# noorgme/Decentralised-Verification-and-Distributed-Execution-of-Large-Scale-Video-Diffusion-Models

Measured on AMD Instinct MI355X. Metric: denoising steps/sec, Zeroscope-XL 24f@1024x576 (CFG UNet3D forward + guidance + DDIM), higher is better.
Workload: dtype f16

## Files before the change

### decentralised-verification-and-distributed-execution-of-large-scale-video-diffusion-models_amd/_lib.py

```python
from __future__ import annotations

import ctypes as C
import os

_HERE = os.path.dirname(os.path.abspath(__file__))
LIB_PATH = os.environ.get("VDX_LIB_PATH") or os.path.join(_HERE, "libvdx_hip.so")


class GemmArgs(C.Structure):
    _fields_ = [
        ("a", C.c_void_p), ("a2", C.c_void_p), ("w", C.c_void_p), ("bias", C.c_void_p),
        ("bias2", C.c_void_p), ("residual", C.c_void_p), ("out", C.c_void_p),
        ("M", C.c_int32), ("N", C.c_int32), ("K", C.c_int32), ("mode", C.c_int32),
        ("c1", C.c_int32), ("c2", C.c_int32),
        ("lda", C.c_int32), ("lda2", C.c_int32), ("ldo", C.c_int32), ("ldr", C.c_int32),
        ("h_in", C.c_int32), ("w_in", C.c_int32), ("h_out", C.c_int32), ("w_out", C.c_int32),
        ("stride", C.c_int32), ("upsample", C.c_int32), ("frames", C.c_int32), ("hw", C.c_int32),
        ("rows_per_bias2", C.c_int32), ("ldb2", C.c_int32), ("epilogue", C.c_int32),
        ("row_begin", C.c_int32), ("row_end", C.c_int32),
        ("ksplit", C.c_int32), ("wset_rows", C.c_int32), ("workspace", C.c_void_p), ("wset_bias", C.c_void_p),
        ("workspace_bytes", C.c_size_t), ("pad_mode", C.c_int32),
    ]


class ClipPreprocessArgs(C.Structure):
    _fields_ = [
        ("frames", C.c_void_p), ("x_bounds", C.c_void_p), ("x_coeffs", C.c_void_p), ("y_bounds", C.c_void_p),
        ("y_coeffs", C.c_void_p), ("out", C.c_void_p), ("out_u8", C.c_void_p),
        ("frame_pitch", C.c_size_t), ("row_pitch", C.c_int32), ("F", C.c_int32), ("H", C.c_int32), ("W", C.c_int32),
        ("kx", C.c_int32), ("ky", C.c_int32), ("band", C.c_int32), ("span", C.c_int32), ("ldo", C.c_int32),
    ]


class TomeArgs(C.Structure):
    _fields_ = [
        ("src_idx", C.c_void_p), ("dst_idx", C.c_void_p), ("inv", C.c_void_p), ("node_max", C.c_void_p),
        ("node_idx", C.c_void_p), ("slot", C.c_void_p), ("off", C.c_void_p), ("items", C.c_void_p),
        ("n_img", C.c_int32), ("S", C.c_int32), ("n_src", C.c_int32), ("n_dst", C.c_int32), ("r", C.c_int32), ("C", C.c_int32),
    ]


_vp, _i, _f, _sz = C.c_void_p, C.c_int, C.c_float, C.c_size_t

SIGNATURES = {
    "vdx_last_error": (C.c_char_p, []),
    "vdx_version": (_i, []),
    "vdx_build_flags": (_i, []),
    "vdx_gemm_f16": (_i, [C.POINTER(GemmArgs), _vp]),
    "vdx_gemm_plan": (_i, [C.POINTER(GemmArgs), C.POINTER(C.c_int32), C.POINTER(C.c_int32)]),
    "vdx_gemm_kernel_name": (_i, [C.POINTER(GemmArgs), C.c_char_p, _sz]),
    "vdx_gemm_plan_ksplit": (_i, [C.POINTER(GemmArgs), C.POINTER(C.c_int32), C.POINTER(C.c_int32), C.POINTER(C.c_size_t)]),
    "vdx_softmax_rows_f16": (_i, [_vp, _i, _i, _i, _f, _vp]),
    "vdx_rows_to_u8_frames": (_i, [_vp, _i, _sz, _vp, _vp]),
    "vdx_im2col_in_f16": (_i, [_vp, _vp, _i, _i, _i, _i, _i, _i, _vp]),
    "vdx_rows_to_ncfhw_f16": (_i, [_vp, _i, _vp, _i, _i, _i, _i, _i, _vp]),
    "vdx_silu_f16": (_i, [_vp, _vp, _sz, _vp]),
    "vdx_groupnorm_workspace": (_sz, [_i, _i, _i, _i]),
    "vdx_groupnorm_f16": (_i, [_vp, _i, _i, _vp, _i, _i, _vp, _vp, _f, _i, _i, _i, _i, _vp, _i, _vp, _vp]),
    "vdx_groupnorm_workspace_part": (_sz, [_i, _i, _i, _i, _i]),
    "vdx_groupnorm_part_f16": (_i, [_vp, _i, _i, _vp, _i, _i, _vp, _vp, _f, _i, _i, _i, _i, _vp, _i, _vp, _i, _vp]),
    "vdx_groupnorm_fold_linear_f16": (_i, [_vp, _i, _i, _vp, _vp, _f, _i, _i, _i, _vp, _i, _vp, _vp, _i, _vp, _vp, _vp]),
    "vdx_groupnorm_stats_f16": (_i, [_vp, _i, _i, _vp, _i, _i, _vp, _vp, _f, _i, _i, _i, _vp, _i, C.POINTER(_sz), _vp]),
    "vdx_conv3x3_gn_supported": (_i, [_i, _i, _i]),
    "vdx_conv3x3_gn_preferred": (_i, [_i, _i, _i, _i, _i, _i]),
    "vdx_conv3x3_gn_f16": (_i, [_vp, _i, _vp, _i, _i, _i, _vp, _vp, _vp, _vp, _i, _i, _vp, _i, _vp, _i, _i, _i, _i, _i, _vp]),
    "vdx_tconv_gn_supported": (_i, [_i, _i, _i]),
    "vdx_tconv_gn_preferred": (_i, [_i, _i, _i, _i, _i]),
    "vdx_tconv_gn_f16": (_i, [_vp, _i, _vp, _vp, _vp, _vp, _i, _vp, _i, _i, _i, _i, _i, _i, _vp]),
    "vdx_layernorm_f16": (_i, [_vp, _i, _vp, _vp, _f, _i, _i, _vp, _i, _vp]),
    "vdx_flash_attn_f16": (_i, [_vp, _i, _vp, _i, _vp, _i, _vp, _i, _i, _i, _i, _i, _i, _i, _f, _i, _vp]),
    "vdx_flash_attn_rows_f16": (_i, [_vp, _i, _vp, _i, _vp, _i, _vp, _i, _i, _i, _i, _i, _i, _i, _f, _i, _vp]),
    "vdx_timestep_embedding_f16": (_i, [_vp, _vp, _i, _i, _vp]),
    "vdx_gelu_f16": (_i, [_vp, _vp, _sz, _vp]),
    "vdx_temporal_attn_f16": (_i, [_vp, _i, _vp, _i, _i, _i, _i, _i, _f, _vp]),
    "vdx_ff_block_supported": (_i, [_i]),
    "vdx_ff_block_pack_bytes": (_sz, [_i]),
    "vdx_ff_block_f16": (_i, [_vp, _i, _vp, _f, _vp, _i, _i, _i, _vp]),
    "vdx_ff_block_proj_pack_bytes": (_sz, [_i]),
    "vdx_ff_block_proj_f16": (_i, [_vp, _i, _vp, _f, _vp, _i, _i, _vp, _vp, _i, _i, _i, _vp]),
    "vdx_cross_attn_block_supported": (_i, [_i, _i]),
    "vdx_cross_attn_block_pack_bytes": (_sz, [_i]),
    "vdx_cross_attn_block_kv_bytes": (_sz, [_i]),
    "vdx_cross_attn_block_f16": (_i, [_vp, _i, _vp, _vp, _i, _f, _vp, _i, _i, _i, _i, _vp]),
    "vdx_temporal_attn_block_supported": (_i, [_i, _i]),
    "vdx_temporal_attn_block_wqkv_bytes": (_sz, [_i]),
    "vdx_temporal_attn_block_wo_bytes": (_sz, [_i]),
    "vdx_temporal_attn_block_f16": (_i, [_vp, _i, _vp, _vp, _f, _vp, _vp, _vp, _vp, _i, _i, _i, _i, _i, _f, _vp]),
    "vdx_temporal_attn_block2_supported": (_i, [_i, _i]),
    "vdx_temporal_attn_block2_pack_bytes": (_sz, [_i]),
    "vdx_temporal_attn_block2_f16": (_i, [_vp, _i, _vp, _f, _vp, _i, _i, _i, _i, _i, _vp]),
    "vdx_comm_unique_id": (_i, [_vp]),
    "vdx_comm_init": (_i, [_vp, _i, _i, C.POINTER(_vp)]),
    "vdx_comm_destroy": (_i, [_vp]),
    "vdx_allgather_shard": (_i, [_vp, _vp, _vp, _sz, _vp]),
    "vdx_halo_exchange": (_i, [_vp, _vp, _sz, _i, _vp, _sz, _i, _vp]),
    "vdx_ipc_export": (_i, [_vp, _vp, C.POINTER(_sz)]),
    "vdx_ipc_open": (_i, [_vp, _sz, C.POINTER(_vp)]),
    "vdx_ipc_close": (_i, [_vp, _sz]),
    "vdx_peer_gather": (_i, [_vp, C.POINTER(_vp), _i, _sz, _vp]),
    "vdx_set_reserved_cus": (_i, [_i]),
    "vdx_reserved_cus": (_i, []),
    "vdx_persistent_grid_cus": (_i, []),
    "vdx_probe_mfma_f16": (_i, [_vp, _sz, _i, C.POINTER(C.c_double), _vp]),
    "vdx_probe_occupancy_hog": (_i, [_i, _i, _i, _vp]),
    "vdx_cfg_input_f16": (_i, [_vp, _vp, _f, _vp, _i, _i, _i, _vp]),
    "vdx_cfg_ddim_step_f16": (_i, [_vp, _vp, _vp, _f, _f, _f, _f, _f, _sz, _vp]),
    "vdx_ddim_step_f16": (_i, [_vp, _vp, _vp, _f, _f, _f, _f, _sz, _vp]),
    "vdx_cfg_dpm_step_f16": (_i, [_vp, _vp, _vp, _vp, _vp, _f, _f, _f, _f, _f, _f, _f, _sz, _vp]),
    "vdx_dpm_step_f16": (_i, [_vp, _vp, _vp, _vp, _vp, _f, _f, _f, _f, _f, _f, _sz, _vp]),
    "vdx_blend_accumulate_f16": (_i, [_vp, _vp, _vp, _vp, _i, _i, _i, _i, _i, _vp]),
    "vdx_blend_finalize_f32": (_i, [_vp, _vp, _vp, _i, _i, _i, _vp]),
    "vdx_clip_preprocess_u8": (_i, [C.POINTER(ClipPreprocessArgs), _vp]),
    "vdx_clip_vision_embed_f16": (_i, [_vp, _i, _vp, _vp, _vp, _vp, _f, _i, _i, _i, _i, _vp, _i, _vp]),
# ... 156 lines not shown
```

### decentralised-verification-and-distributed-execution-of-large-scale-video-diffusion-models_amd/csrc/norm.hip

```cpp
#include "vdx_common.h"

static int gn_rows_for(int n_samples, int rows_per_sample, int min_blocks) {
    int rows = 128;
    while (rows > 8 && (long long)n_samples * ((rows_per_sample + rows - 1) / rows) < min_blocks) rows >>= 1;
    return rows;
}
static int gn_stat_rows(int n_samples, int rows_per_sample) { return gn_rows_for(n_samples, rows_per_sample, 256); }

struct GnP {
    const f16 *x, *x2;
    int c1, c2, ldx, ldx2;
    int C, G, cpg, nvec, krows;
    int n_samples, rps, nslabs, slab_rows;
    int apply_rows;
    float* partial;
    float* ab;
};

__device__ __forceinline__ f16x8 gn_load(const GnP& p, size_t row, int cv) {
    const int c = cv * 8;
    const f16* src = c < p.c1 ? p.x + row * p.ldx + c : p.x2 + row * p.ldx2 + (c - p.c1);
    return *(const f16x8*)src;
}

struct Moments {
    float n, mean, m2;
};
__device__ __forceinline__ Moments merge(const Moments a, const Moments b) {
    if (b.n == 0.f) return a;
    if (a.n == 0.f) return b;
    const float n = a.n + b.n, d = b.mean - a.mean;
    return Moments{n, a.mean + d * (b.n / n), a.m2 + b.m2 + d * d * (a.n * b.n / n)};
}

__global__ void gn_partial_kernel(const GnP p) {
    extern __shared__ float lds[];
    const int tid = threadIdx.x;
    const int sample = blockIdx.y, slab = blockIdx.x;
    const int cv = tid % p.nvec, rsub = tid / p.nvec;
    float k[8], s[8], ss[8];
#pragma unroll
    for (int j = 0; j < 8; ++j) k[j] = s[j] = ss[j] = 0.f;
    const int r_end = min(p.rps, (slab + 1) * p.slab_rows);
    const size_t base = (size_t)sample * p.rps;
    int cnt = 0;
    int r = slab * p.slab_rows + rsub;
    auto acc = [&](const f16x8 v) {
#pragma unroll
        for (int j = 0; j < 8; ++j) {
            const float f = (float)v[j] - k[j];
            s[j] += f;
            ss[j] += f * f;
        }
// ... 108 lines not shown
__global__ void gn_apply_kernel(const GnP p, f16* y, int ldy) {
    const int tid = threadIdx.x;
    const int sample = blockIdx.y, slab = blockIdx.x;
    const int cv = tid % p.nvec, rsub = tid / p.nvec;
    float a[8], b[8];
    const float* ab = p.ab + ((size_t)sample * p.C + cv * 8) * 2;
#pragma unroll
    for (int j = 0; j < 8; ++j) {
        a[j] = ab[2 * j];
        b[j] = ab[2 * j + 1];
    }
    const int r_end = min(p.rps, (slab + 1) * p.apply_rows);
    const size_t base = (size_t)sample * p.rps;
    for (int r = slab * p.apply_rows + rsub; r < r_end; r += p.krows) {
        const size_t row = base + r;
        const f16x8 v = gn_load(p, row, cv);
        f16x8 o;
#pragma unroll
        for (int j = 0; j < 8; ++j) {
            float f = (float)v[j] * a[j] + b[j];
            if (SILU) f = silu_f(f);
            o[j] = (f16)f;
        }
        *(f16x8*)(y + row * ldy + cv * 8) = o;
    }
}

static int gn_threads(int nvec, int* krows) {
    int k = nvec >= 256 ? 1 : (256 + nvec - 1) / nvec;
    *krows = k;
    return k * nvec;
}

extern "C" size_t vdx_groupnorm_workspace_part(int n_samples, int rows_per_sample, int C, int G, int partition_samples) {
    const int rows = gn_stat_rows(partition_samples > 0 ? partition_samples : n_samples, rows_per_sample);
    const size_t nslabs = (rows_per_sample + rows - 1) / rows;
    return ((((size_t)n_samples * nslabs * G * 3 + 3) & ~(size_t)3) + (size_t)n_samples * C * 2) * sizeof(float);
}
extern "C" size_t vdx_groupnorm_workspace(int n_samples, int rows_per_sample, int C, int G) {
    return vdx_groupnorm_workspace_part(n_samples, rows_per_sample, C, G, 0);
}

extern "C" int vdx_groupnorm_part_f16(const void* x, int c1, int ldx, const void* x2, int c2, int ldx2,
                                      const void* gamma, const void* beta, float eps, int G,
                                      int n_samples, int rows_per_sample, int silu, void* y, int ldy,
                                      void* workspace, int partition_samples, vdx_stream_t stream);
extern "C" int vdx_groupnorm_f16(const void* x, int c1, int ldx, const void* x2, int c2, int ldx2,
                                 const void* gamma, const void* beta, float eps, int G,
                                 int n_samples, int rows_per_sample, int silu, void* y, int ldy,
                                 void* workspace, vdx_stream_t stream) {
    return vdx_groupnorm_part_f16(x, c1, ldx, x2, c2, ldx2, gamma, beta, eps, G, n_samples, rows_per_sample, silu, y, ldy,
                                  workspace, 0, stream);
}
static int gn_run(const void* x, int c1, int ldx, const void* x2, int c2, int ldx2,
                  const void* gamma, const void* beta, float eps, int G,
                  int n_samples, int rows_per_sample, int silu, void* y, int ldy,
                  void* workspace, int partition_samples, bool stats_only, GnP& p, vdx_stream_t stream) {
    VDX_CHECK(x && gamma && beta && (y || stats_only) && workspace, "groupnorm: null pointer");
    const int C = c1 + c2;
    VDX_CHECK(c1 > 0 && c1 % 8 == 0 && c2 % 8 == 0, "groupnorm: c1=%d c2=%d must be multiples of 8", c1, c2);
    VDX_CHECK((c2 == 0) == (x2 == nullptr), "groupnorm: x2/c2 mismatch");
    VDX_CHECK(G > 0 && C % G == 0, "groupnorm: C=%d not divisible by G=%d", C, G);
    VDX_CHECK(ldx % 8 == 0 && ldy % 8 == 0 && (c2 == 0 || ldx2 % 8 == 0), "groupnorm: leading dims must be multiples of 8");
    VDX_CHECK(n_samples > 0 && rows_per_sample > 0, "groupnorm: empty input");
    VDX_CHECK(C / 8 <= 1024, "groupnorm: C=%d too wide", C);
    p.x = (const f16*)x; p.x2 = (const f16*)x2; p.c1 = c1; p.c2 = c2; p.ldx = ldx; p.ldx2 = ldx2;
    p.C = C; p.G = G; p.cpg = C / G; p.nvec = C / 8;
    p.n_samples = n_samples; p.rps = rows_per_sample;
    p.slab_rows = gn_stat_rows(partition_samples > 0 ? partition_samples : n_samples, rows_per_sample);
    p.apply_rows = gn_rows_for(n_samples, rows_per_sample, 1024);
    p.nslabs = (rows_per_sample + p.slab_rows - 1) / p.slab_rows;
    p.partial = (float*)workspace;
    p.ab = p.partial + (((size_t)n_samples * p.nslabs * G * 3 + 3) & ~(size_t)3);
    const int nt = gn_threads(p.nvec, &p.krows);
    hipStream_t st = (hipStream_t)stream;
    dim3 grid(p.nslabs, n_samples);
    hipLaunchKernelGGL(gn_partial_kernel, grid, dim3(nt), (2 * (size_t)p.krows * C + p.krows + 2 * (size_t)G * p.krows) * sizeof(float), st, p);
    const int nsg = n_samples * G;
    hipLaunchKernelGGL(gn_finalize_kernel, dim3((nsg + 3) / 4), dim3(256), 0, st, p, (const f16*)gamma, (const f16*)beta, eps);
    if (stats_only) return vdx_launch_status("vdx_groupnorm_f16 (statistics)");
    dim3 agrid((rows_per_sample + p.apply_rows - 1) / p.apply_rows, n_samples);
    if (silu)
        hipLaunchKernelGGL(gn_apply_kernel<true>, agrid, dim3(nt), 0, st, p, (f16*)y, ldy);
    else
        hipLaunchKernelGGL(gn_apply_kernel<false>, agrid, dim3(nt), 0, st, p, (f16*)y, ldy);
    return vdx_launch_status("vdx_groupnorm_f16");
}
extern "C" int vdx_groupnorm_part_f16(const void* x, int c1, int ldx, const void* x2, int c2, int ldx2,
                                      const void* gamma, const void* beta, float eps, int G,
                                      int n_samples, int rows_per_sample, int silu, void* y, int ldy,
                                      void* workspace, int partition_samples, vdx_stream_t stream) {
    GnP p;
    return gn_run(x, c1, ldx, x2, c2, ldx2, gamma, beta, eps, G, n_samples, rows_per_sample, silu, y, ldy, workspace,
                  partition_samples, false, p, stream);
}

extern "C" int vdx_groupnorm_stats_f16(const void* x, int c1, int ldx, const void* x2, int c2, int ldx2, const void* gamma,
                                       const void* beta, float eps, int G, int n_samples, int rows_per_sample, void* workspace,
                                       int partition_samples, size_t* scale_shift_offset, vdx_stream_t stream) {
    VDX_CHECK(scale_shift_offset, "groupnorm_stats: null pointer");
    GnP p;
    if (const int rc = gn_run(x, c1, ldx, x2, c2, ldx2, gamma, beta, eps, G, n_samples, rows_per_sample, 0, nullptr, 0, workspace,
                              partition_samples, true, p, stream))
        return rc;
    *scale_shift_offset = (size_t)((const char*)p.ab - (const char*)workspace);
    return 0;
}

__global__ void gn_fold_kernel(const float* ab, const f16* beta, const f16* w, const f16* bias, int C, int N, int n_samples,
                               f16* w_out, float* bias_out) {
    const int lane = threadIdx.x & 63;
    const long long sn = (long long)blockIdx.x * (blockDim.x >> 6) + (threadIdx.x >> 6);
    if (sn >= (long long)n_samples * N) return;
    const int sample = (int)(sn / N), n = (int)(sn % N);
    const float* abs_ = ab + (size_t)sample * C * 2;
    const f16* wr = w + (size_t)n * C;
    f16* wo = w_out + ((size_t)sample * N + n) * C;
    float acc = 0.f;
    for (int c = lane; c < C; c += 64) {
        const float a = abs_[2 * c], b = abs_[2 * c + 1], wv = (float)wr[c], be = (float)beta[c];
        const f16 w16 = (f16)(wv * a);
        wo[c] = w16;
        const float mean = a != 0.f ? (be - b) / a : 0.f;
        acc += wv * be - (float)w16 * mean;
    }
    acc = wave_sum(acc);
    if (lane == 0) bias_out[(size_t)sample * N + n] = acc + (bias ? (float)bias[n] : 0.f);
}

extern "C" int vdx_groupnorm_fold_linear_f16(const void* x, int C, int ldx, const void* gamma, const void* beta, float eps, int G,
                                             int n_samples, int rows_per_sample, void* workspace, int partition_samples,
                                             const void* w, const void* bias, int N, void* w_out, void* bias_out,
                                             vdx_stream_t stream) {
    VDX_CHECK(w && w_out && bias_out, "groupnorm_fold_linear: null pointer");
    VDX_CHECK(N > 0 && (long long)n_samples * N < (1ll << 31), "groupnorm_fold_linear: bad N");
    GnP p;
    if (const int rc = gn_run(x, C, ldx, nullptr, 0, 0, gamma, beta, eps, G, n_samples, rows_per_sample, 0, nullptr, 0, workspace,
                              partition_samples, true, p, stream))
        return rc;
    const long long waves = (long long)n_samples * N;
    hipLaunchKernelGGL(gn_fold_kernel, dim3((unsigned)((waves + 3) / 4)), dim3(256), 0, (hipStream_t)stream, p.ab, (const f16*)beta,
                       (const f16*)w, (const f16*)bias, C, N, n_samples, (f16*)w_out, (float*)bias_out);
    return vdx_launch_status("vdx_groupnorm_fold_linear_f16");
}

template <int NV>
__global__ __launch_bounds__(256) void layernorm_kernel(const f16* x, int ldx, const f16* gamma, const f16* beta,
                                                         float eps, int M, int C, f16* y, int ldy) {
    const int lane = threadIdx.x & 63;
    const int row = blockIdx.x * 4 + (threadIdx.x >> 6);
    if (row >= M) return;
    const int nvec = C >> 3;
    const f16* xr = x + (size_t)row * ldx;
    f16x8 v[NV];
    float s = 0.f;
#pragma unroll
    for (int i = 0; i < NV; ++i) {
        const int cv = lane + 64 * i;
        if (cv < nvec) {
            v[i] = *(const f16x8*)(xr + cv * 8);
#pragma unroll
            for (int j = 0; j < 8; ++j) s += (float)v[i][j];
        }
    }
    const float mean = wave_sum(s) / (float)C;
    float q = 0.f;
#pragma unroll
    for (int i = 0; i < NV; ++i) {
        if (lane + 64 * i < nvec) {
#pragma unroll
            for (int j = 0; j < 8; ++j) {
                const float d = (float)v[i][j] - mean;
                q += d * d;
            }
        }
    }
    const float rstd = rsqrtf(wave_sum(q) / (float)C + eps);
    f16* yr = y + (size_t)row * ldy;
#pragma unroll
    for (int i = 0; i < NV; ++i) {
        const int cv = lane + 64 * i;
        if (cv < nvec) {
            const f16x8 g = *(const f16x8*)(gamma + cv * 8);
            const f16x8 b = *(const f16x8*)(beta + cv * 8);
            f16x8 o;
#pragma unroll
            for (int j = 0; j < 8; ++j) o[j] = (f16)(((float)v[i][j] - mean) * rstd * (float)g[j] + (float)b[j]);
            *(f16x8*)(yr + cv * 8) = o;
        }
    }
}

template <int CTRL>
__device__ __forceinline__ float dpp_add(float v) {
    return v + __builtin_bit_cast(float, __builtin_amdgcn_update_dpp(0, __builtin_bit_cast(int, v), CTRL, 0xF, 0xF, false));
}
// ... 191 lines not shown
```

### decentralised-verification-and-distributed-execution-of-large-scale-video-diffusion-models_amd/ops.py

```python
from __future__ import annotations

import contextlib
import ctypes as C
from typing import NamedTuple, Optional, Tuple

import torch

from . import _lib
from ._lib import GemmArgs, VdxError
from .frames import is_packed

PLAIN, CONV3X3, TCONV3 = 0, 1, 2
EPI_GEGLU = 1


def _stream() -> int:
    return torch.cuda.current_stream().cuda_stream


def _p(t: Optional[torch.Tensor], name: str, dtype=torch.float16) -> Optional[int]:
    if t is None:
        return None
    if not t.is_cuda:
        raise VdxError(f"{name}: expected a GPU tensor (the denoising path has no CPU fallback)")
# ... 372 lines not shown


def clip_preprocess(frames, out=None, return_u8=False):
    F, H, W = check_u8_frames(frames, "clip_preprocess")
    if pillow_resizes_vertically_first(H, W, CLIP_IMAGE):
        frames, H = resize_u8(frames, CLIP_IMAGE, W, "bilinear"), CLIP_IMAGE
    dev = frames.device
    xb, xk, _ = _clip_table(W, dev)
    yb, yk, yb_host = _clip_table(H, dev)
    band = CLIP_BAND
    while band > 1 and clip_band_span(yb_host, band) * CLIP_IMAGE * 3 > CLIP_LDS_MAX:
        band //= 2
    span = clip_band_span(yb_host, band)
    if span * CLIP_IMAGE * 3 > CLIP_LDS_MAX:
        raise VdxError(f"clip_preprocess: H={H} needs {span} input rows per output row (more than LDS holds)")
    out, ldo = _out(out, F * 49, 3072, frames, "clip_preprocess")
    u8 = torch.empty((F, CLIP_IMAGE, CLIP_IMAGE, 3), dtype=torch.uint8, device=dev) if return_u8 else None
    a = _lib.ClipPreprocessArgs()
    a.frames, a.frame_pitch, a.row_pitch = _u8_args(frames)
    a.out, a.out_u8 = _p(out, "out"), (u8.data_ptr() if u8 is not None else None)
    a.x_bounds, a.x_coeffs, a.y_bounds, a.y_coeffs = xb.data_ptr(), xk.data_ptr(), yb.data_ptr(), yk.data_ptr()
    a.F, a.H, a.W = F, H, W
    a.kx, a.ky, a.band, a.span, a.ldo = xk.shape[1], yk.shape[1], band, span, ldo
    _launch("vdx_clip_preprocess_u8", C.byref(a))
    return (out, u8) if return_u8 else out


def clip_vision_embed(patch, class_emb, pos_emb, gamma, beta, *, F, seq_pad, eps=1e-5, out=None):
    r, D, ldp = _rows(patch, "patch")
    P = pos_emb.shape[0] - 1
    if r < F * P or pos_emb.shape[1] != D or class_emb.numel() != D or gamma.numel() != D or beta.numel() != D:
        raise VdxError(f"clip_vision_embed: patch [{r}][{D}], pos {tuple(pos_emb.shape)}: shapes do not match F={F}")
    if seq_pad <= P or not pos_emb.is_contiguous():
        raise VdxError(f"clip_vision_embed: seq_pad={seq_pad} must exceed {P} patches; pos_emb contiguous")
    out, ldo = _out(out, F * seq_pad, D, patch, "clip_vision_embed")
    _launch("vdx_clip_vision_embed_f16", _p(patch, "patch"), ldp, _p(class_emb, "class_emb"), _p(pos_emb, "pos_emb"),
            _p(gamma, "gamma"), _p(beta, "beta"), float(eps), F, P, seq_pad, D, _p(out, "out"), ldo)
    return out


def clip_cosine_score(img, txt):
    F, D, ldi = _rows(img, "img")
    if txt.numel() != D or not txt.is_contiguous():
        raise VdxError(f"clip_cosine_score: text embedding has {txt.numel()} values, images {D}")
    if F == 0:
        raise VdxError("clip_cosine_score: no frames")
    per = torch.empty(F, dtype=torch.float32, device=img.device)
    mean = torch.empty(1, dtype=torch.float32, device=img.device)
    _launch("vdx_clip_cosine_score_f16", _p(img, "img"), ldi, _p(txt, "txt"), F, D, _p(per, "per_frame", torch.float32),
            _p(mean, "mean", torch.float32))
    return mean, per


def groupnorm(x, gamma, beta, *, groups, n_samples, rows_per_sample, eps, silu_act, x2=None, out=None, partition_samples=0):
    r, c1, ldx = _rows(x, "x")
    c2, ldx2 = 0, 0
    M = n_samples * rows_per_sample
    if r < M:
        raise VdxError(f"groupnorm: x has {r} rows, need {M}")
    if x2 is not None:
        r2, c2, ldx2 = _rows(x2, "x2")
        if r2 < M:
            raise VdxError(f"groupnorm: x2 has {r2} rows, need {M}")
    Cc = c1 + c2
    if gamma.numel() != Cc or beta.numel() != Cc:
        raise VdxError(f"groupnorm: gamma/beta size {gamma.numel()} != C={Cc}")
    out, ldy = _out(out, M, Cc, x, "groupnorm")
    need = _lib.load().vdx_groupnorm_workspace_part(n_samples, rows_per_sample, Cc, groups, partition_samples)
    ws = _scratch(_GN_WS, x.device, need, torch.uint8, 1 << 20)
    _launch("vdx_groupnorm_part_f16", _p(x, "x"), c1, ldx, _p(x2, "x2"), c2, ldx2, _p(gamma, "gamma"), _p(beta, "beta"),
            float(eps), groups, n_samples, rows_per_sample, int(bool(silu_act)), _p(out, "out"), ldy, ws.data_ptr(),
            partition_samples)
    return out


def conv3x3_gn_preferred(c1: int, c2: int, N: int, n_img: int, h: int, w: int) -> bool:
    return bool(_lib.load().vdx_conv3x3_gn_preferred(c1, c2, N, n_img, h, w))


def conv3x3_gn_supported(c1: int, c2: int, N: int) -> bool:
    return bool(_lib.load().vdx_conv3x3_gn_supported(c1, c2, N))


def conv3x3_gn(x, gamma, beta, w, *, x2=None, bias=None, bias2=None, rows_per_bias2=0, residual=None, groups, n_img, h, wd, eps,
               partition_samples=0, out=None):
    r, c1, ldx = _rows(x, "x")
    S = h * wd
    M = n_img * S
    c2 = ldx2 = 0
    if x2 is not None:
        r2, c2, ldx2 = _rows(x2, "x2")
        if r2 < M:
            raise VdxError(f"conv3x3_gn: x2 has {r2} rows, need {M}")
    Cc = c1 + c2
    N, K = w.shape
    if r < M or K != 9 * Cc or gamma.numel() != Cc or beta.numel() != Cc or not w.is_contiguous():
        raise VdxError(f"conv3x3_gn: x [{r}][{c1}] (+{c2}), w [{N}][{K}], gamma {gamma.numel()}, M = {M}: shapes do not match")
    if not conv3x3_gn_supported(c1, c2, N):
        raise VdxError(f"conv3x3_gn: c1={c1}, c2={c2}, N={N} not supported")
    if bias is not None and bias.numel() != N:
        raise VdxError(f"conv3x3_gn: bias has {bias.numel()} elements, N={N}")
    ldb2 = _covers(bias2, M, N, "conv3x3_gn", "bias2", rows_per_bias2)
    ldr = _covers(residual, M, N, "conv3x3_gn", "residual")
    out, ldo = _out(out, M, N, x, "conv3x3_gn")
    need = _lib.load().vdx_groupnorm_workspace_part(n_img, S, Cc, groups, partition_samples)
    ws = _scratch(_GN_WS, x.device, need, torch.uint8, 1 << 20)
# ... 1722 lines not shown
```

### include/vdx.h

```cpp
#ifndef VDX_H
#define VDX_H
#include <stddef.h>
#include <stdint.h>

#ifdef __cplusplus
extern "C" {
#endif

typedef void* vdx_stream_t;

const char* vdx_last_error(void);
int vdx_version(void);
int vdx_build_flags(void);

enum { VDX_GEMM_PLAIN = 0, VDX_GEMM_CONV3X3 = 1, VDX_GEMM_TCONV3 = 2 };
enum { VDX_EPI_GEGLU = 1 };

typedef struct vdx_gemm_args {
    const void* a;
    const void* a2;
    const void* w;
    const void* bias;
    const void* bias2;
    const void* residual;
    void* out;
    int32_t M, N, K;
    int32_t mode;
    int32_t c1, c2;
    int32_t lda, lda2, ldo, ldr;
    int32_t h_in, w_in;
    int32_t h_out, w_out;
    int32_t stride;
    int32_t upsample;
    int32_t frames, hw;
    int32_t rows_per_bias2, ldb2;
    int32_t epilogue;
    int32_t row_begin, row_end;
    int32_t ksplit;
    int32_t wset_rows;
    void* workspace;
    const float* wset_bias;
    size_t workspace_bytes;
    int32_t pad_mode;
} vdx_gemm_args;

int vdx_gemm_f16(const vdx_gemm_args* a, vdx_stream_t stream);

int vdx_gemm_plan(const vdx_gemm_args* a, int32_t* variant, int32_t* split_row);
int vdx_gemm_kernel_name(const vdx_gemm_args* a, char* buf, size_t n);
int vdx_gemm_plan_ksplit(const vdx_gemm_args* a, int32_t* split_row, int32_t* ksplit, size_t* workspace_bytes);

int vdx_im2col_in_f16(const void* x_ncfhw, void* out_rows, int B, int Cin, int F, int H, int W,
                      int Kpad, vdx_stream_t stream);

int vdx_rows_to_ncfhw_f16(const void* rows, int ld, void* out, int B, int C, int F, int H, int W,
                          vdx_stream_t stream);

int vdx_silu_f16(const void* x, void* y, size_t n, vdx_stream_t stream);

int vdx_timestep_embedding_f16(const float* t_device, void* out, int B, int dim, vdx_stream_t stream);

int vdx_gelu_f16(const void* x, void* y, size_t n, vdx_stream_t stream);

size_t vdx_groupnorm_workspace(int n_samples, int rows_per_sample, int C, int G);
int vdx_groupnorm_f16(const void* x, int c1, int ldx, const void* x2, int c2, int ldx2,
                      const void* gamma, const void* beta, float eps, int G,
                      int n_samples, int rows_per_sample, int silu,
                      void* y, int ldy, void* workspace, vdx_stream_t stream);
size_t vdx_groupnorm_workspace_part(int n_samples, int rows_per_sample, int C, int G, int partition_samples);
int vdx_groupnorm_fold_linear_f16(const void* x, int C, int ldx, const void* gamma, const void* beta, float eps, int G,
                                  int n_samples, int rows_per_sample, void* workspace, int partition_samples,
                                  const void* w, const void* bias, int N, void* w_out, void* bias_out, vdx_stream_t stream);
int vdx_groupnorm_part_f16(const void* x, int c1, int ldx, const void* x2, int c2, int ldx2,
                           const void* gamma, const void* beta, float eps, int G,
                           int n_samples, int rows_per_sample, int silu,
                           void* y, int ldy, void* workspace, int partition_samples, vdx_stream_t stream);
int vdx_groupnorm_stats_f16(const void* x, int c1, int ldx, const void* x2, int c2, int ldx2, const void* gamma,
                            const void* beta, float eps, int G, int n_samples, int rows_per_sample, void* workspace,
                            int partition_samples, size_t* scale_shift_offset, vdx_stream_t stream);
int vdx_conv3x3_gn_supported(int c1, int c2, int N);
int vdx_conv3x3_gn_preferred(int c1, int c2, int N, int n_img, int h, int w);
int vdx_conv3x3_gn_f16(const void* a, int lda, const void* a2, int lda2, int c1, int c2, const float* scale_shift,
                       const void* w, const void* bias, const void* bias2, int rows_per_bias2, int ldb2,
                       const void* residual, int ldr, void* out, int ldo, int n_img, int h, int w_px, int N,
                       vdx_stream_t stream);
int vdx_tconv_gn_supported(int C, int N, int F);
int vdx_tconv_gn_preferred(int C, int N, int B, int F, int S);
int vdx_tconv_gn_f16(const void* x, int ldx, const float* scale_shift, const void* w, const void* bias,
                     const void* residual, int ldr, void* out, int ldo, int B, int F, int S, int C, int N,
                     vdx_stream_t stream);
int vdx_softmax_rows_f16(void* x, int ld, int rows, int cols, float scale, vdx_stream_t stream);

int vdx_layernorm_f16(const void* x, int ldx, const void* gamma, const void* beta, float eps,
                      int M, int C, void* y, int ldy, vdx_stream_t stream);

int vdx_flash_attn_f16(const void* q, int ldq, const void* k, int ldk, const void* vt, int ldvt,
                       void* out, int ldo, int n_seq, int sq, int skv, int skv_pad, int heads,
                       int seq_per_kv, float scale, int causal, vdx_stream_t stream);
int vdx_flash_attn_rows_f16(const void* q, int ldq, const void* k, int ldk, const void* v, int ldv,
                            void* out, int ldo, int n_seq, int sq, int skv, int skv_pad, int heads,
                            int seq_per_kv, float scale, int causal, vdx_stream_t stream);

int vdx_ff_block_supported(int inner);
size_t vdx_ff_block_pack_bytes(int inner);
int vdx_ff_block_f16(const void* t, int ldt, const void* packed, float eps, void* out, int ldo, int M, int inner,
                     vdx_stream_t stream);
size_t vdx_ff_block_proj_pack_bytes(int inner);
int vdx_ff_block_proj_f16(const void* t, int ldt, const void* packed, float eps, const void* x, int ldx, int xrows,
                          const void* proj_packed, void* out, int ldo, int M, int inner, vdx_stream_t stream);

int vdx_temporal_attn_f16(const void* qkv, int ldqkv, void* out, int ldo, int B, int F, int HW,
                          int heads, float scale, vdx_stream_t stream);

int vdx_temporal_attn_block_supported(int inner, int F);
size_t vdx_temporal_attn_block_wqkv_bytes(int inner);
size_t vdx_temporal_attn_block_wo_bytes(int inner);
int vdx_temporal_attn_block_f16(const void* t, int ldt, const void* gamma, const void* beta, float eps,
                                const void* wqkv_packed, const void* wo_packed, const void* bo,
                                void* out, int ldo, int B, int F, int HW, int inner, float scale,
                                vdx_stream_t stream);

int vdx_cross_attn_block_supported(int inner, int kv_len);
size_t vdx_cross_attn_block_pack_bytes(int inner);
size_t vdx_cross_attn_block_kv_bytes(int inner);
int vdx_cross_attn_block_f16(const void* t, int ldt, const void* packed, const void* kv_packed, int kv_len, float eps,
                             void* out, int ldo, int n_items, int rows_per_item, int inner, vdx_stream_t stream);

int vdx_temporal_attn_block2_supported(int inner, int F);
size_t vdx_temporal_attn_block2_pack_bytes(int inner);
// ... 314 lines not shown
```

Baseline: 6.300.

## Add single-pass LDS-resident groupnorm kernel and route eligible shapes to it

Adds a groupnorm kernel that runs one block per (sample, group). The block loads the whole group slab into LDS, computes statistics with a hierarchical Welford-style merge, and applies the normalisation (with optional SiLU) from LDS. This replaces the multi-kernel stats-then-apply path, whose extra launches, workspace traffic and second global read of the input it aims to remove. Routing is on by default for shapes whose LDS footprint allows two blocks per CU. It reserves up to 160 KB of LDS, which can limit occupancy, and only (sample, group) blocks provide parallelism.

```diff
diff --git a/decentralised-verification-and-distributed-execution-of-large-scale-video-diffusion-models_amd/_lib.py b/decentralised-verification-and-distributed-execution-of-large-scale-video-diffusion-models_amd/_lib.py
--- a/decentralised-verification-and-distributed-execution-of-large-scale-video-diffusion-models_amd/_lib.py
+++ b/decentralised-verification-and-distributed-execution-of-large-scale-video-diffusion-models_amd/_lib.py
@@ -59,6 +59,11 @@
     "vdx_groupnorm_f16": (_i, [_vp, _i, _i, _vp, _i, _i, _vp, _vp, _f, _i, _i, _i, _i, _vp, _i, _vp, _vp]),
     "vdx_groupnorm_workspace_part": (_sz, [_i, _i, _i, _i, _i]),
     "vdx_groupnorm_part_f16": (_i, [_vp, _i, _i, _vp, _i, _i, _vp, _vp, _f, _i, _i, _i, _i, _vp, _i, _vp, _i, _vp]),
+    "vdx_groupnorm_onepass_supported": (_i, [_i, _i, _i, _i, _i]),
+    "vdx_groupnorm_onepass_preferred": (_i, [_i, _i, _i, _i, _i]),
+    "vdx_set_groupnorm_onepass": (None, [_i]),
+    "vdx_groupnorm_onepass_launches": (_sz, []),
+    "vdx_groupnorm_onepass_f16": (_i, [_vp, _i, _i, _vp, _i, _i, _vp, _vp, _f, _i, _i, _i, _i, _vp, _i, _i, _vp]),
     "vdx_groupnorm_fold_linear_f16": (_i, [_vp, _i, _i, _vp, _vp, _f, _i, _i, _i, _vp, _i, _vp, _vp, _i, _vp, _vp, _vp]),
     "vdx_groupnorm_stats_f16": (_i, [_vp, _i, _i, _vp, _i, _i, _vp, _vp, _f, _i, _i, _i, _vp, _i, C.POINTER(_sz), _vp]),
     "vdx_conv3x3_gn_supported": (_i, [_i, _i, _i]),
diff --git a/decentralised-verification-and-distributed-execution-of-large-scale-video-diffusion-models_amd/csrc/norm.hip b/decentralised-verification-and-distributed-execution-of-large-scale-video-diffusion-models_amd/csrc/norm.hip
--- a/decentralised-verification-and-distributed-execution-of-large-scale-video-diffusion-models_amd/csrc/norm.hip
+++ b/decentralised-verification-and-distributed-execution-of-large-scale-video-diffusion-models_amd/csrc/norm.hip
@@ -1,4 +1,6 @@
 #include "vdx_common.h"
+#include <atomic>
+#include <stdlib.h>
 
 static int gn_rows_for(int n_samples, int rows_per_sample, int min_blocks) {
     int rows = 128;
@@ -213,6 +215,11 @@
     return vdx_groupnorm_part_f16(x, c1, ldx, x2, c2, ldx2, gamma, beta, eps, G, n_samples, rows_per_sample, silu, y, ldy,
                                   workspace, 0, stream);
 }
+static bool gn1_routed(int c1, int c2, int G, int rows_per_sample, int part_samples);
+extern "C" int vdx_groupnorm_onepass_f16(const void* x, int c1, int ldx, const void* x2, int c2, int ldx2,
+                                         const void* gamma, const void* beta, float eps, int G,
+                                         int n_samples, int rows_per_sample, int silu, void* y, int ldy,
+                                         int partition_samples, vdx_stream_t stream);
 static int gn_run(const void* x, int c1, int ldx, const void* x2, int c2, int ldx2,
                   const void* gamma, const void* beta, float eps, int G,
                   int n_samples, int rows_per_sample, int silu, void* y, int ldy,
@@ -251,6 +258,9 @@
                                       const void* gamma, const void* beta, float eps, int G,
                                       int n_samples, int rows_per_sample, int silu, void* y, int ldy,
                                       void* workspace, int partition_samples, vdx_stream_t stream) {
+    if (gn1_routed(c1, c2, G, rows_per_sample, partition_samples > 0 ? partition_samples : n_samples))
+        return vdx_groupnorm_onepass_f16(x, c1, ldx, x2, c2, ldx2, gamma, beta, eps, G, n_samples, rows_per_sample, silu, y, ldy,
+                                         partition_samples, stream);
     GnP p;
     return gn_run(x, c1, ldx, x2, c2, ldx2, gamma, beta, eps, G, n_samples, rows_per_sample, silu, y, ldy, workspace,
                   partition_samples, false, p, stream);
@@ -303,6 +313,253 @@
     hipLaunchKernelGGL(gn_fold_kernel, dim3((unsigned)((waves + 3) / 4)), dim3(256), 0, (hipStream_t)stream, p.ab, (const f16*)beta,
                        (const f16*)w, (const f16*)bias, C, N, n_samples, (f16*)w_out, (float*)bias_out);
     return vdx_launch_status("vdx_groupnorm_fold_linear_f16");
+}
+
+struct Gn1P {
+    const f16 *x, *x2, *gamma, *beta;
+    f16* y;
+    int c1, c2, ldx, ldx2, ldy;
+    int G, cpg, nv;
+    int rps, nslabs, slab_rows, krows;
+    int rpar;
+    float eps;
+};
+
+static size_t gn1_lds_bytes(int rps, int cpg, int nslabs, int krows) {
+    const size_t T = (size_t)nslabs * krows;
+    return (((size_t)rps * cpg * 2 + 15) & ~(size_t)15) + (2 * T * cpg + 3 * T + 3 * (size_t)nslabs + 2 * (size_t)cpg) * sizeof(float);
+}
+
+template <int V, bool SILU>
+__global__ __launch_bounds__(1024) void gn_onepass_kernel(const Gn1P p) {
+#pragma clang fp contract(off)
+    typedef f16 vec __attribute__((ext_vector_type(V)));
+    extern __shared__ __attribute__((aligned(16))) unsigned char gn1_lds[];
+    const int tid = threadIdx.x, nt = blockDim.x;
+    const int lid = xcd_remap(blockIdx.x, gridDim.x);
+    const int sample = lid / p.G, g = lid - sample * p.G;
+    const int W = p.cpg, T = p.nslabs * p.krows;
+    f16* slab = (f16*)gn1_lds;
+    float* tm = (float*)(gn1_lds + (((size_t)p.rps * W * 2 + 15) & ~(size_t)15));
+    float* tq = tm + T * W;
+    float* cn = tq + T * W;
+    float* tmp = cn + T;
+    float* part = tmp + 2 * T;
+    float* ab = part + 3 * p.nslabs;
+
+    const int vc = tid % p.nv, r0 = tid / p.nv;
+    const bool active = r0 < p.rpar;
+    const int ch = g * W + vc * V;
+    const bool first = ch < p.c1;
+    const size_t ld = first ? p.ldx : p.ldx2;
+    const f16* src = (first ? p.x + ch : p.x2 + (ch - p.c1)) + (size_t)sample * p.rps * ld;
+    if (active) {
+        for (int r = r0; r < p.rps; r += 4 * p.rpar) {
+            vec v[4];
+#pragma unroll
+            for (int u = 0; u < 4; ++u) v[u] = *(const vec*)(src + (size_t)min(r + u * p.rpar, p.rps - 1) * ld);
+#pragma unroll
+            for (int u = 0; u < 4; ++u)
+                if (r + u * p.rpar < p.rps) *(vec*)(slab + (r + u * p.rpar) * W + vc * V) = v[u];
+        }
+    }
+    __syncthreads();
+    for (int ci = tid; ci < T * W; ci += nt) {
+        const int t = ci / W, c = ci - t * W;
+        const int sl = t / p.krows, rs = t - sl * p.krows;
+        const int r_end = min(p.rps, (sl + 1) * p.slab_rows);
+        int r = sl * p.slab_rows + rs, cnt = 0;
+        float k = 0.f, s = 0.f, ss = 0.f;
+        if (r < r_end) k = (float)slab[r * W + c];
+        auto acc = [&](const f16 v) {
+            const float f = (float)v - k;
+            s = s + f;
+            ss = __builtin_fmaf(f, f, ss);
+        };
+        for (; r + 3 * p.krows < r_end; r += 4 * p.krows, cnt += 4) {
+            const f16 v0 = slab[r * W + c], v1 = slab[(r + p.krows) * W + c];
+            const f16 v2 = slab[(r + 2 * p.krows) * W + c], v3 = slab[(r + 3 * p.krows) * W + c];
+            acc(v0); acc(v1); acc(v2); acc(v3);
+        }
+        for (; r < r_end; r += p.krows, ++cnt) acc(slab[r * W + c]);
+        const float inv = cnt ? 1.0f / (float)cnt : 0.f;
+        tm[ci] = __builtin_fmaf(s, inv, k);
+        tq[ci] = __builtin_fmaf(-inv, s * s, ss);
+        if (c == 0) cn[t] = (float)cnt;
+    }
+    __syncthreads();
+    for (int i = tid; i < T; i += nt) {
+        const float *mp = tm + i * W, *qp = tq + i * W;
+        float ms = 0.f, qs = 0.f;
+        for (int c = 0; c < W; ++c) {
+            ms = ms + mp[c];
+            qs = qs + qp[c];
+        }
+        const float mean = ms / (float)W;
+        float dev = 0.f;
+        for (int c = 0; c < W; ++c) {
+            const float d = mp[c] - mean;
+            dev = __builtin_fmaf(d, d, dev);
+        }
+        tmp[2 * i] = mean;
+        tmp[2 * i + 1] = __builtin_fmaf(dev, cn[i], qs);
+    }
+    __syncthreads();
+    for (int sl = tid; sl < p.nslabs; sl += nt) {
+        float an = 0.f, am = 0.f, aq = 0.f;
+        for (int rs = 0; rs < p.krows; ++rs) {
+            const int i = sl * p.krows + rs;
+            const float bn = cn[i] * (float)W, bm = tmp[2 * i], bq = tmp[2 * i + 1];
+            if (bn == 0.f) continue;
+            if (an == 0.f) {
+                an = bn; am = bm; aq = bq;
+                continue;
+            }
+            const float n = an + bn, d = bm - am;
+            am = __builtin_fmaf(d, bn / n, am);
+            aq = __builtin_fmaf(an * bn / n, d * d, aq + bq);
+            an = n;
+        }
+        part[3 * sl] = an;
+        part[3 * sl + 1] = am;
+        part[3 * sl + 2] = aq;
+    }
+    __syncthreads();
+    if (tid < 64) {
+        const int lane = tid;
+        const double K = (double)part[1];
+        double N = 0.0, S1 = 0.0, S2 = 0.0, Q = 0.0;
+        for (int i = lane; i < p.nslabs; i += 64) {
+            const double nn = (double)part[3 * i], d = (double)part[3 * i + 1] - K;
+            N = N + nn;
+            S1 = __builtin_fma(d, nn, S1);
+            S2 = __builtin_fma(d, d * nn, S2);
+            Q = Q + (double)part[3 * i + 2];
+        }
+#pragma unroll
+        for (int o = 32; o > 0; o >>= 1) {
+            const double Nb = __shfl_xor(N, o, 64), S1b = __shfl_xor(S1, o, 64), S2b = __shfl_xor(S2, o, 64), Qb = __shfl_xor(Q, o, 64);
+            const bool low = (lane & o) == 0;
+            N = low ? N + Nb : Nb + N;
+            S1 = low ? S1 + S1b : S1b + S1;
+            S2 = low ? S2 + S2b : S2b + S2;
+            Q = low ? Q + Qb : Qb + Q;
+        }
+        const double mean = N > 0.0 ? K + S1 / N : 0.0, m2 = N > 0.0 ? Q + S2 - S1 * S1 / N : 0.0;
+        double var = N > 0.0 ? m2 / N : 0.0;
+        if (var < 0.0) var = 0.0;
+        const float rstd = (float)(1.0 / sqrt(var + (double)p.eps));
+        for (int j = lane; j < W; j += 64) {
+            const float a = rstd * (float)p.gamma[g * W + j];
+            ab[2 * j] = a;
+            ab[2 * j + 1] = __builtin_fmaf(-(float)mean, a, (float)p.beta[g * W + j]);
+        }
+    }
+    __syncthreads();
+    if (active) {
+        float a[V], b[V];
+#pragma unroll
+        for (int j = 0; j < V; ++j) {
+            a[j] = ab[2 * (vc * V + j)];
+            b[j] = ab[2 * (vc * V + j) + 1];
+        }
+        f16* dst = p.y + (size_t)sample * p.rps * p.ldy + ch;
+        for (int r = r0; r < p.rps; r += p.rpar) {
+            const vec v = *(const vec*)(slab + r * W + vc * V);
+            vec o;
+#pragma unroll
+            for (int j = 0; j < V; ++j) {
+                float f = __builtin_fmaf((float)v[j], a[j], b[j]);
+                if (SILU) f = silu_f(f);
+                o[j] = (f16)f;
+            }
+            *(vec*)(dst + (size_t)r * p.ldy) = o;
+        }
+    }
+}
+
+static bool gn1_plan(int c1, int c2, int G, int rows_per_sample, int part_samples, Gn1P& p, int* vwidth, size_t* lds) {
+    const int C = c1 + c2;
+    if (c1 <= 0 || c2 < 0 || c1 % 8 || c2 % 8 || G <= 0 || C % G || rows_per_sample <= 0 || part_samples <= 0 || C / 8 > 1024) return false;
+    const int cpg = C / G;
+    const int V = cpg % 8 == 0 ? 8 : cpg % 4 == 0 ? 4 : cpg % 2 == 0 ? 2 : 0;
+    if (!V || (long long)rows_per_sample * cpg * 2 > 163840) return false;
+    p.G = G; p.cpg = cpg; p.nv = cpg / V; p.rps = rows_per_sample;
+    p.slab_rows = gn_stat_rows(part_samples, rows_per_sample);
+    p.nslabs = (rows_per_sample + p.slab_rows - 1) / p.slab_rows;
+    gn_threads(C / 8, &p.krows);
+    *lds = gn1_lds_bytes(rows_per_sample, cpg, p.nslabs, p.krows);
+    *vwidth = V;
+    return *lds <= 163840 && p.nv <= 256;
+}
+
+extern "C" int vdx_groupnorm_onepass_supported(int c1, int c2, int G, int rows_per_sample, int partition_samples) {
+    Gn1P p;
+    int V;
+    size_t lds;
+    return gn1_plan(c1, c2, G, rows_per_sample, partition_samples, p, &V, &lds) ? 1 : 0;
+}
+
+extern "C" int vdx_groupnorm_onepass_preferred(int c1, int c2, int G, int rows_per_sample, int partition_samples) {
+    Gn1P p;
+    int V;
+    size_t lds;
+    return gn1_plan(c1, c2, G, rows_per_sample, partition_samples, p, &V, &lds) && 2 * lds <= 163840 ? 1 : 0;
+}
+
+static int gn1_env_mode() {
+    const char* e = getenv("VDX_GN_ONEPASS");
+    return e && e[0] == '0' && !e[1] ? 0 : e && e[0] == '1' && !e[1] ? 1 : -1;
+}
+static std::atomic<int> g_gn1_mode{-2};
+static std::atomic<size_t> g_gn1_launches{0};
+extern "C" void vdx_set_groupnorm_onepass(int mode) { g_gn1_mode = mode == 0 || mode == 1 || mode == -1 ? mode : -2; }
+extern "C" size_t vdx_groupnorm_onepass_launches() { return g_gn1_launches; }
+static bool gn1_routed(int c1, int c2, int G, int rows_per_sample, int part_samples) {
+    static const int env_mode = gn1_env_mode();
+    int mode = g_gn1_mode;
+    if (mode == -2) mode = env_mode;
+    if (mode == 0) return false;
+    return mode == 1 ? vdx_groupnorm_onepass_supported(c1, c2, G, rows_per_sample, part_samples)
+                     : vdx_groupnorm_onepass_preferred(c1, c2, G, rows_per_sample, part_samples);
+}
+
+template <int V>
+static int gn1_launch(const Gn1P& p, int silu, int blocks, int nt, size_t lds, hipStream_t st) {
+    static const hipError_t attr_rc = vdx_reserve_lds(163840, gn_onepass_kernel<V, true>, gn_onepass_kernel<V, false>);
+    if (attr_rc != hipSuccess) return vdx_fail("groupnorm_onepass: cannot reserve 160 KB of LDS");
+    if (silu)
+        hipLaunchKernelGGL((gn_onepass_kernel<V, true>), dim3(blocks), dim3(nt), lds, st, p);
+    else
+        hipLaunchKernelGGL((gn_onepass_kernel<V, false>), dim3(blocks), dim3(nt), lds, st, p);
+    return vdx_launch_status("vdx_groupnorm_onepass_f16");
+}
+
+extern "C" int vdx_groupnorm_onepass_f16(const void* x, int c1, int ldx, const void* x2, int c2, int ldx2,
+                                         const void* gamma, const void* beta, float eps, int G,
+                                         int n_samples, int rows_per_sample, int silu, void* y, int ldy,
+                                         int partition_samples, vdx_stream_t stream) {
+    VDX_CHECK(x && gamma && beta && y, "groupnorm_onepass: null pointer");
+    VDX_CHECK((c2 == 0) == (x2 == nullptr), "groupnorm_onepass: x2/c2 mismatch");
+    VDX_CHECK(ldx % 8 == 0 && ldy % 8 == 0 && (c2 == 0 || ldx2 % 8 == 0), "groupnorm_onepass: leading dims must be multiples of 8");
+    VDX_CHECK(n_samples > 0 && (long long)n_samples * G < (1ll << 31), "groupnorm_onepass: bad n_samples=%d", n_samples);
+    Gn1P p;
+    int V;
+    size_t lds;
+    VDX_CHECK(gn1_plan(c1, c2, G, rows_per_sample, partition_samples > 0 ? partition_samples : n_samples, p, &V, &lds),
+              "groupnorm_onepass: c1=%d c2=%d G=%d rows_per_sample=%d not supported", c1, c2, G, rows_per_sample);
+    VDX_CHECK(ldx >= c1 && ldx2 >= c2 && ldy >= c1 + c2, "groupnorm_onepass: leading dims below the widths");
+    p.x = (const f16*)x; p.x2 = (const f16*)x2; p.gamma = (const f16*)gamma; p.beta = (const f16*)beta; p.y = (f16*)y;
+    p.c1 = c1; p.c2 = c2; p.ldx = ldx; p.ldx2 = ldx2; p.ldy = ldy; p.eps = eps;
+    const int per_cu = (int)(163840 / lds);
+    int nt = 1024;
+    while (nt > 256 && (nt * per_cu > 2048 || (long long)p.nv * rows_per_sample <= nt / 2)) nt >>= 1;
+    p.rpar = nt / p.nv;
+    hipStream_t st = (hipStream_t)stream;
+    const int blocks = n_samples * G;
+    ++g_gn1_launches;
+    return V == 8 ? gn1_launch<8>(p, silu, blocks, nt, lds, st) : V == 4 ? gn1_launch<4>(p, silu, blocks, nt, lds, st)
+                                                                         : gn1_launch<2>(p, silu, blocks, nt, lds, st);
 }
 
 template <int NV>
diff --git a/decentralised-verification-and-distributed-execution-of-large-scale-video-diffusion-models_amd/ops.py b/decentralised-verification-and-distributed-execution-of-large-scale-video-diffusion-models_amd/ops.py
--- a/decentralised-verification-and-distributed-execution-of-large-scale-video-diffusion-models_amd/ops.py
+++ b/decentralised-verification-and-distributed-execution-of-large-scale-video-diffusion-models_amd/ops.py
@@ -448,6 +448,22 @@
     return mean, per
 
 
+def set_groupnorm_onepass(mode: Optional[bool]) -> None:
+    _lib.load().vdx_set_groupnorm_onepass(-2 if mode is None else int(bool(mode)))
+
+
+def groupnorm_onepass_launches() -> int:
+    return int(_lib.load().vdx_groupnorm_onepass_launches())
+
+
+def groupnorm_onepass_supported(C: int, C2: int, groups: int, rows_per_sample: int, n_samples: int = 0) -> bool:
+    return bool(_lib.load().vdx_groupnorm_onepass_supported(C - C2, C2, groups, rows_per_sample, n_samples or 256))
+
+
+def groupnorm_onepass_preferred(C: int, C2: int, groups: int, rows_per_sample: int, n_samples: int = 0) -> bool:
+    return bool(_lib.load().vdx_groupnorm_onepass_preferred(C - C2, C2, groups, rows_per_sample, n_samples or 256))
+
+
 def groupnorm(x, gamma, beta, *, groups, n_samples, rows_per_sample, eps, silu_act, x2=None, out=None, partition_samples=0):
     r, c1, ldx = _rows(x, "x")
     c2, ldx2 = 0, 0
diff --git a/include/vdx.h b/include/vdx.h
--- a/include/vdx.h
+++ b/include/vdx.h
@@ -75,6 +75,14 @@
                            const void* gamma, const void* beta, float eps, int G,
                            int n_samples, int rows_per_sample, int silu,
                            void* y, int ldy, void* workspace, int partition_samples, vdx_stream_t stream);
+int vdx_groupnorm_onepass_supported(int c1, int c2, int G, int rows_per_sample, int partition_samples);
+int vdx_groupnorm_onepass_preferred(int c1, int c2, int G, int rows_per_sample, int partition_samples);
+void vdx_set_groupnorm_onepass(int mode);
+size_t vdx_groupnorm_onepass_launches(void);
+int vdx_groupnorm_onepass_f16(const void* x, int c1, int ldx, const void* x2, int c2, int ldx2,
+                              const void* gamma, const void* beta, float eps, int G,
+                              int n_samples, int rows_per_sample, int silu,
+                              void* y, int ldy, int partition_samples, vdx_stream_t stream);
 int vdx_groupnorm_stats_f16(const void* x, int c1, int ldx, const void* x2, int c2, int ldx2, const void* gamma,
                             const void* beta, float eps, int G, int n_samples, int rows_per_sample, void* workspace,
                             int partition_samples, size_t* scale_shift_offset, vdx_stream_t stream);
```

New measurement: 6.317 (median of 6 runs). Within noise of the previous version (+0.3%).
